# ErlerPhilipp/points2surf

Measured on NVIDIA H100. Metric: SDF queries/sec at grid_res=256, higher is better.
Workload: dtype f16 operands / f32 accumulate (wgmma); hi/lo split f16 (fp32-level) for FC tails and guard-band recompute

## Files before the change

### points2surf_b200/csrc/net_tc.cu

```cuda
#include "model.cuh"
#include "tc_ptx.cuh"

namespace p2s {

using namespace ptx;

namespace {

constexpr int kTile = 64;
constexpr int kWG = 2;
constexpr int kThreads = 128 * kWG;
template <bool PRECISE>
struct Cfg {
    static constexpr int kChunks = PRECISE ? 2 : 4;
    static constexpr int kSplit = 8 / kChunks;
    static constexpr uint32_t kChunkBytes = PRECISE ? 65536u : 32768u;
    static constexpr uint32_t kW3Bytes = kChunks * kChunkBytes;
    static constexpr uint32_t kMidScale = PRECISE ? 2u : 1u;
    static constexpr uint32_t kMidBytes = (8192u + 8192u + 16384u) * kMidScale;
    static constexpr uint32_t kPerqBytes = PRECISE ? 16384u : 8192u;
    static constexpr uint32_t kRedBytes = 4u * kChunks * 128u * 4u;
    static constexpr uint32_t kOffMid = kW3Bytes;
    static constexpr uint32_t kWgWq = kPerqBytes;
    static constexpr uint32_t kWgBytes = kWgWq + 192 * 4;
    static constexpr uint32_t kOffWg = kOffMid + kMidBytes;
    static constexpr uint32_t kOffBias = kOffWg + kWG * kWgBytes;
    static constexpr uint32_t kSlotBytes = PRECISE ? 0u : 8u * 128u * 16u;
    static constexpr uint32_t kOffSlot = kOffBias + 320 * 4;
    static constexpr uint32_t kOffXBar = kOffSlot + kWG * kSlotBytes;
    static constexpr uint32_t kSmemBytes = kOffXBar + (PRECISE ? 0u : kWG * 16u);
};
static_assert(Cfg<false>::kSmemBytes <= 232448 && Cfg<true>::kSmemBytes <= 232448, "shared memory budget");
static_assert(Cfg<false>::kRedBytes <= Cfg<false>::kPerqBytes && Cfg<true>::kRedBytes <= Cfg<true>::kPerqBytes, "reduction scratch");

struct Seg {
    const float* ptr;
    int n;
    int tiles;
    int center;
};

struct PassParams {
    Seg seg[2];
    const float* query;
    const float* R;
    int tiles_per_query;
    int B;
    const float* W0;
    const float* b0;
    int num_mid;
    int mid_N[3];
    const uint8_t* mid_img[3];
    const float* mid_bias[3];
    int perq_layer;
    const uint8_t* perq_img;
    const uint8_t* w3_img;
    float* out;
};

__device__ __forceinline__ uint32_t pack_relu(float a, float b) {
    uint32_t r;
    asm("cvt.rn.relu.satfinite.f16x2.f32 %0, %1, %2;" : "=r"(r) : "f"(b), "f"(a));
    return r;
}
__device__ __forceinline__ void pack_relu_split(float a, float b, uint32_t& hi, uint32_t& lo) {
    hi = pack_relu(a, b);
    const float2 hf = __half22float2(*reinterpret_cast<const __half2*>(&hi));
    lo = pack_half2(fmaxf(a, 0.f) - hf.x, fmaxf(b, 0.f) - hf.y);
}
template <bool PRECISE>
__device__ __forceinline__ void pack_act(float a, float b, uint32_t& hi, uint32_t& lo) {
    if (PRECISE) pack_relu_split(a, b, hi, lo);
    else hi = pack_relu(a, b);
}

template <bool PRECISE, int R>
__device__ __forceinline__ void mid_mma(float (&d)[R], const uint32_t (&a)[4], const uint32_t (&al)[4], uint64_t w, uint64_t w_lo, uint32_t acc) {
    if (R == 32) {
        auto& d32 = reinterpret_cast<float (&)[32]>(d);
        if (PRECISE) { wgmma_rs_n64(d32, al, w, acc); wgmma_rs_n64(d32, a, w_lo, 1); wgmma_rs_n64(d32, a, w, 1); }
        else wgmma_rs_n64(d32, a, w, acc);
    } else {
        auto& d64 = reinterpret_cast<float (&)[64]>(d);
        if (PRECISE) { wgmma_rs_n128(d64, al, w, acc); wgmma_rs_n128(d64, a, w_lo, 1); wgmma_rs_n128(d64, a, w, 1); }
        else wgmma_rs_n128(d64, a, w, acc);
    }
}

template <bool PRECISE, int R, int KL>
__device__ __forceinline__ void pack_acc(const float (&d)[R], const float* bias, int q4, uint32_t (&a)[R / 8][4], uint32_t (&al)[R / 8][KL]) {
#pragma unroll
    for (int j = 0; j < R / 4; ++j) {
        const float2 bb = *reinterpret_cast<const float2*>(bias + 8 * j + 2 * q4);
        pack_act<PRECISE>(d[4 * j] + bb.x, d[4 * j + 1] + bb.y, a[j >> 1][(j & 1) * 2], al[j >> 1][PRECISE ? (j & 1) * 2 : 0]);
        pack_act<PRECISE>(d[4 * j + 2] + bb.x, d[4 * j + 3] + bb.y, a[j >> 1][(j & 1) * 2 + 1], al[j >> 1][PRECISE ? (j & 1) * 2 + 1 : 0]);
    }
}

template <int S>
__device__ __forceinline__ void max_halve(float (&m)[32], int lane) {
    const bool up = (lane & S) != 0;
#pragma unroll
    for (int i = 0; i < S; ++i) {
        const float send = up ? m[i] : m[i + S], keep = up ? m[i + S] : m[i];
        m[i] = fmaxf(keep, __shfl_xor_sync(0xffffffffu, send, S));
    }
}

template <bool PRECISE>
__global__ void __launch_bounds__(kThreads, 1) pointnet_pass_kernel(const PassParams p) {
    using C = Cfg<PRECISE>;
    constexpr int kL = PRECISE ? 4 : 1;
    extern __shared__ __align__(1024) uint8_t smem[];
    float* s_bias = reinterpret_cast<float*>(smem + C::kOffBias);
    const int tid = threadIdx.x, wg = tid >> 7, t = tid & 127, lane = tid & 31, q4 = lane & 3;
    const int r0 = (t >> 5) * 16 + (lane >> 2);
    const int part = blockIdx.x % C::kSplit;
    const int stream = blockIdx.x / C::kSplit, nstreams = gridDim.x / C::kSplit;
    const int nq = (p.B > stream) ? (p.B - stream + nstreams - 1) / nstreams : 0;
    const int tpq = p.tiles_per_query;
    uint32_t mid_off[3] = {0, 0, 0};
    {
        uint32_t o = 0;
        for (int l = 0; l < (PRECISE ? p.num_mid : 3); ++l) {
            if (!PRECISE && l >= p.num_mid) break;
            mid_off[l] = o; o += (uint32_t)p.mid_N[l] * 128u * C::kMidScale;
        }
    }

    if (nq > 0) {
        const uint4* src = reinterpret_cast<const uint4*>(p.w3_img + (size_t)part * C::kW3Bytes);
        uint4* dst = reinterpret_cast<uint4*>(smem);
        for (uint32_t i = tid; i < C::kW3Bytes / 16; i += kThreads) dst[i] = src[i];
        for (int l = 0; l < (PRECISE ? p.num_mid : 3); ++l) {
            if (!PRECISE && l >= p.num_mid) break;
            if (l == p.perq_layer) continue;
            const uint4* s = reinterpret_cast<const uint4*>(p.mid_img[l]);
            uint4* d = reinterpret_cast<uint4*>(smem + C::kOffMid + mid_off[l]);
            for (uint32_t i = tid; i < (uint32_t)p.mid_N[l] * 8u * C::kMidScale; i += kThreads) d[i] = s[i];
        }
    }
    {
        int off = 0;
        for (int l = 0; l < p.num_mid; ++l) {
            for (int i = tid; i < p.mid_N[l]; i += kThreads) s_bias[off + i] = p.mid_bias[l][i];
            off += p.mid_N[l];
        }
        for (int i = tid; i < 64; i += kThreads) s_bias[256 + i] = p.b0[i];
    }
    uint64_t* xbar = reinterpret_cast<uint64_t*>(smem + C::kOffXBar);
    if (!PRECISE && tid == 0) {
        for (int w = 0; w < kWG; ++w) {
            mbar_init(xbar + 2 * w, 1);
            mbar_arrive_expect_tx(xbar + 2 * w, C::kSlotBytes);
            mbar_init(xbar + 2 * w + 1, 128);
        }
        fence_mbar_init();
    }
    fence_proxy_async_smem();
    __syncthreads();
    if (!PRECISE) cluster_sync();

    uint8_t* wsm = smem + C::kOffWg + wg * C::kWgBytes;
    uint8_t* perq = wsm;
    float* red = reinterpret_cast<float*>(perq);
    float* wq = reinterpret_cast<float*>(wsm + C::kWgWq);
    const float* s_b0 = s_bias + 256;
    const uint32_t bar_id = 1 + (uint32_t)wg;
    auto wg_sync = [&]() { asm volatile("bar.sync %0, 128;" ::"r"(bar_id) : "memory"); };
    const uint64_t dsc_w3 = make_smem_desc(smem_u32(smem), 128, 2048);
    uint64_t dsc_mid[3], dsc_mid_lo[3];
    for (int l = 0; l < 3; ++l) {
        const bool pq = l == p.perq_layer;
        dsc_mid[l] = make_smem_desc(pq ? smem_u32(perq) : smem_u32(smem + C::kOffMid) + mid_off[l], 128, 1024);
        dsc_mid_lo[l] = dsc_mid[l] + (uint64_t)((pq ? 8192u : (uint32_t)p.mid_N[l] * 128u) >> 4);
    }
    uint8_t* slot = smem + C::kOffSlot + wg * C::kSlotBytes;
    uint64_t* full = xbar + 2 * wg;
    uint64_t* empty = xbar + 2 * wg + 1;
    const uint32_t peer = (uint32_t)part ^ 1u;
    uint32_t nsend = 0, nrecv = 0;

    for (int qi = wg; qi < nq; qi += kWG) {
        const size_t q = (size_t)stream + (size_t)qi * nstreams;
        wg_sync();
        if (t < 64) {
            const float w0 = p.W0[t * 3 + 0], w1 = p.W0[t * 3 + 1], w2 = p.W0[t * 3 + 2];
            float r[9] = {1.f, 0.f, 0.f, 0.f, 1.f, 0.f, 0.f, 0.f, 1.f};
            if (p.R) {
#pragma unroll
                for (int i = 0; i < 9; ++i) r[i] = p.R[q * 9 + i];
            }
            wq[0 * 64 + t] = w0 * r[0] + w1 * r[3] + w2 * r[6];
            wq[1 * 64 + t] = w0 * r[1] + w1 * r[4] + w2 * r[7];
            wq[2 * 64 + t] = w0 * r[2] + w1 * r[5] + w2 * r[8];
        }
        if (p.perq_layer >= 0) {
            const uint4* s = reinterpret_cast<const uint4*>(p.perq_img + q * C::kPerqBytes);
            uint4* d = reinterpret_cast<uint4*>(perq);
            for (uint32_t i = t; i < C::kPerqBytes / 16; i += 128) d[i] = s[i];
            fence_proxy_async_smem();
        }
        wg_sync();
        float vmax[4 * C::kChunks];
#pragma unroll
        for (int i = 0; i < 4 * C::kChunks; ++i) vmax[i] = -INFINITY;
        const int own = PRECISE ? 0 : (part ^ wg ^ (qi >> 1)) & 1;
        for (int i = 0; i < tpq; ++i) {
            const int tq = PRECISE ? i : (i & ~1) + own;
            const bool mine = PRECISE || (!(i & 1) && tq < tpq);
            uint32_t a2[8][4], a2l[8][kL];
            if (mine) {
                const int sgi = tq < p.seg[0].tiles ? 0 : 1;
                const Seg& sg = p.seg[sgi];
                float cx = 0.f, cy = 0.f, cz = 0.f;
                if (sg.center) { cx = p.query[q * 3 + 0]; cy = p.query[q * 3 + 1]; cz = p.query[q * 3 + 2]; }
                float px[2], py[2], pz[2];
#pragma unroll
                for (int h = 0; h < 2; ++h) {
                    int local = (tq - (sgi ? p.seg[0].tiles : 0)) * kTile + r0 + 8 * h;
                    if (local >= sg.n) local = 0;
                    const float* src = sg.ptr + (q * sg.n + local) * 3;
                    px[h] = src[0] - cx; py[h] = src[1] - cy; pz[h] = src[2] - cz;
                }
                uint32_t a[4][4], al[4][kL];
#pragma unroll
                for (int kk = 0; kk < 4; ++kk) {
#pragma unroll
                    for (int hc = 0; hc < 2; ++hc) {
                        const int ch = kk * 16 + hc * 8 + 2 * q4;
                        const float2 wx = *reinterpret_cast<const float2*>(wq + 0 * 64 + ch);
                        const float2 wy = *reinterpret_cast<const float2*>(wq + 1 * 64 + ch);
                        const float2 wz = *reinterpret_cast<const float2*>(wq + 2 * 64 + ch);
                        const float2 bb = *reinterpret_cast<const float2*>(s_b0 + ch);
#pragma unroll
                        for (int h = 0; h < 2; ++h) {
                            const float v0 = fmaf(wx.x, px[h], fmaf(wy.x, py[h], fmaf(wz.x, pz[h], bb.x)));
                            const float v1 = fmaf(wx.y, px[h], fmaf(wy.y, py[h], fmaf(wz.y, pz[h], bb.y)));
                            pack_act<PRECISE>(v0, v1, a[kk][hc * 2 + h], al[kk][PRECISE ? hc * 2 + h : 0]);
                        }
                    }
                }
                const float* bl = s_bias;
#pragma unroll
                for (int l = 0; l < 2; ++l) {
                    if (l >= p.num_mid - 1) break;
                    float d[32];
#pragma unroll
                    for (int i = 0; i < 32; ++i) d[i] = 0.f;
                    wgmma_fence();
#pragma unroll
                    for (int ks = 0; ks < 4; ++ks)
                        mid_mma<PRECISE>(d, a[ks], reinterpret_cast<const uint32_t (&)[4]>(al[PRECISE ? ks : 0]), dsc_mid[l] + (uint64_t)(ks * 16), dsc_mid_lo[l] + (uint64_t)(ks * 16), ks > 0);
                    wgmma_commit();
                    wgmma_wait<0>();
                    fence_regs(d);
                    pack_acc<PRECISE>(d, bl, q4, a, al);
                    bl += 64;
                }
                {
                    const uint64_t w = p.num_mid == 3 ? dsc_mid[2] : dsc_mid[0], w_lo = p.num_mid == 3 ? dsc_mid_lo[2] : dsc_mid_lo[0];
                    float d[64];
#pragma unroll
                    for (int i = 0; i < 64; ++i) d[i] = 0.f;
                    wgmma_fence();
#pragma unroll
                    for (int ks = 0; ks < 4; ++ks)
                        mid_mma<PRECISE>(d, a[ks], reinterpret_cast<const uint32_t (&)[4]>(al[PRECISE ? ks : 0]), w + (uint64_t)(ks * 16), w_lo + (uint64_t)(ks * 16), ks > 0);
                    wgmma_commit();
                    wgmma_wait<0>();
                    fence_regs(d);
                    pack_acc<PRECISE>(d, bl, q4, a2, a2l);
                }
                if (!PRECISE) {
                    if (nsend > 0) mbar_wait_cluster_bounded(empty, (nsend - 1) & 1);
                    const uint32_t dst = mapa(smem_u32(slot), peer) + 16u * (uint32_t)t, bar = mapa(smem_u32(full), peer);
#pragma unroll
                    for (int k = 0; k < 8; ++k) st_async_v4(dst + 2048u * k, a2[k], bar);
                    ++nsend;
                }
            } else {
                mbar_wait_cluster_bounded(full, nrecv & 1);
#pragma unroll
                for (int k = 0; k < 8; ++k) {
                    const uint4 v = reinterpret_cast<const uint4*>(slot)[128 * k + t];
                    a2[k][0] = v.x; a2[k][1] = v.y; a2[k][2] = v.z; a2[k][3] = v.w;
                }
                mbar_arrive_cluster(mapa(smem_u32(empty), peer));
                if (t == 0) mbar_arrive_expect_tx(full, C::kSlotBytes);
                ++nrecv;
            }
#pragma unroll(PRECISE ? 1 : C::kChunks)
            for (int c = 0; c < C::kChunks; ++c) {
                float d[64];
#pragma unroll
                for (int i = 0; i < 64; ++i) d[i] = 0.f;
                const uint64_t w = dsc_w3 + (uint64_t)((uint32_t)c * (C::kChunkBytes >> 4));
                wgmma_fence();
#pragma unroll
                for (int ks = 0; ks < 8; ++ks) {
                    const uint64_t o = w + (uint64_t)(ks * 16);
                    if (PRECISE) {
                        wgmma_rs_n128(d, a2[ks], o + (uint64_t)(32768u >> 4), ks > 0);
                        wgmma_rs_n128(d, reinterpret_cast<const uint32_t (&)[4]>(a2l[PRECISE ? ks : 0]), o, 1);
                        wgmma_rs_n128(d, a2[ks], o, 1);
                    } else {
                        wgmma_rs_n128(d, a2[ks], o, ks > 0);
                    }
                }
                wgmma_commit();
                wgmma_wait<0>();
                fence_regs(d);
                float m[32];
#pragma unroll
                for (int j = 0; j < 16; ++j) {
                    m[2 * j] = fmaxf(d[4 * j], d[4 * j + 2]);
                    m[2 * j + 1] = fmaxf(d[4 * j + 1], d[4 * j + 3]);
                }
                max_halve<16>(m, lane);
                max_halve<8>(m, lane);
                max_halve<4>(m, lane);
                float v[4];
#pragma unroll
                for (int i = 0; i < 4; ++i) v[i] = fmaxf(vmax[i], m[i]);
#pragma unroll
                for (int i = 0; i < 4 * (C::kChunks - 1); ++i) vmax[i] = vmax[i + 4];
#pragma unroll
                for (int i = 0; i < 4; ++i) vmax[4 * (C::kChunks - 1) + i] = v[i];
            }
        }
        constexpr int kC = C::kChunks * 128;
        const int warp = t >> 5;
        wg_sync();
#pragma unroll
        for (int c = 0; c < C::kChunks; ++c)
#pragma unroll
            for (int h = 0; h < 2; ++h)
                *reinterpret_cast<float2*>(red + warp * kC + c * 128 + 16 * (lane >> 2) + 8 * h + 2 * q4) = make_float2(vmax[4 * c + 2 * h], vmax[4 * c + 2 * h + 1]);
        wg_sync();
        for (int i = t; i < kC / 4; i += 128) {
            const float4* r4 = reinterpret_cast<const float4*>(red);
            float4 v = r4[i];
#pragma unroll
            for (int w = 1; w < 4; ++w) {
                const float4 u = r4[w * (kC / 4) + i];
                v = make_float4(fmaxf(v.x, u.x), fmaxf(v.y, u.y), fmaxf(v.z, u.z), fmaxf(v.w, u.w));
            }
            *reinterpret_cast<float4*>(p.out + q * 1024 + (size_t)(part * kC + 4 * i)) = v;
        }
    }
    if (!PRECISE) cluster_sync();
}

__global__ void pack_kmajor_kernel(const float* __restrict__ W, int rows, int K, int row0, uint32_t sbo, uint8_t* __restrict__ img, int lo) {
    int e = blockIdx.x * blockDim.x + threadIdx.x;
    if (e >= rows * K) return;
    int r = e / K, k = e % K;
    uint32_t off = (uint32_t)(r >> 3) * sbo + (uint32_t)(k >> 3) * 128u + (uint32_t)(r & 7) * 16u + (uint32_t)(k & 7) * 2u;
    const float w = W[(size_t)(row0 + r) * K + k];
    const __half h = __float2half_rn(w);
    *reinterpret_cast<__half*>(img + off) = lo ? __float2half_rn(w - __half2float(h)) : h;
}

__global__ void pack_perq_kernel(const float* __restrict__ W, int64_t B, uint8_t* __restrict__ img) {
    int64_t e = (int64_t)blockIdx.x * blockDim.x + threadIdx.x;
    if (e >= B * 4096) return;
    int64_t b = e >> 12;
    int r = (int)((e >> 6) & 63), k = (int)(e & 63);
    uint32_t off = (uint32_t)(r >> 3) * 1024u + (uint32_t)(k >> 3) * 128u + (uint32_t)(r & 7) * 16u + (uint32_t)(k & 7) * 2u;
    *reinterpret_cast<__half*>(img + b * 8192 + off) = __float2half_rn(W[e]);
}

__global__ void __launch_bounds__(256) fold_w1_kernel(const float* __restrict__ W1, const float* __restrict__ T, int64_t B, uint8_t* __restrict__ img) {
    __shared__ float sW[64][65];
    __shared__ __align__(16) float sT[64][68];
    const int64_t b = blockIdx.x;
    const int tid = threadIdx.x;
    for (int e = tid; e < 4096; e += 256) {
        const int r = e >> 6, c = e & 63;
        sW[r][c] = W1[e];
        sT[r][c] = T[b * 4096 + e] + (r == c ? 1.0f : 0.0f);
    }
    __syncthreads();
    const int o = tid >> 2, i0 = (tid & 3) * 16;
    float acc[16];
#pragma unroll
    for (int i = 0; i < 16; ++i) acc[i] = 0.f;
    for (int j = 0; j < 64; ++j) {
        const float w = sW[o][j];
#pragma unroll
        for (int i4 = 0; i4 < 4; ++i4) {
            const float4 t4 = *reinterpret_cast<const float4*>(&sT[j][i0 + 4 * i4]);
            acc[4 * i4 + 0] = fmaf(w, t4.x, acc[4 * i4 + 0]);
            acc[4 * i4 + 1] = fmaf(w, t4.y, acc[4 * i4 + 1]);
            acc[4 * i4 + 2] = fmaf(w, t4.z, acc[4 * i4 + 2]);
            acc[4 * i4 + 3] = fmaf(w, t4.w, acc[4 * i4 + 3]);
        }
    }
    uint8_t* dst = img + b * 8192 + (uint32_t)(o >> 3) * 1024u + (uint32_t)(o & 7) * 16u;
#pragma unroll
    for (int h = 0; h < 2; ++h) {
        uint32_t v[4];
#pragma unroll
        for (int e = 0; e < 4; ++e) v[e] = pack_half2(acc[h * 8 + 2 * e], acc[h * 8 + 2 * e + 1]);
        *reinterpret_cast<uint4*>(dst + (uint32_t)(i0 / 8 + h) * 128u) = make_uint4(v[0], v[1], v[2], v[3]);
    }
}

__global__ void fold_fc3_kernel(const float* __restrict__ W1, const float* __restrict__ Wfc3, const float* __restrict__ bfc3,
                                float* __restrict__ G, float* __restrict__ g0) {
    const int oi = blockIdx.x;
    const int o = oi >> 6, i = oi & 63;
    const int k = threadIdx.x;
    float acc = 0.f;
    for (int j = 0; j < 64; ++j) acc = fmaf(W1[o * 64 + j], Wfc3[(size_t)(j * 64 + i) * 256 + k], acc);
    G[(size_t)oi * 256 + k] = acc;
    if (k == 0) {
        float b = W1[o * 64 + i];
        for (int j = 0; j < 64; ++j) b = fmaf(W1[o * 64 + j], bfc3[j * 64 + i], b);
        g0[oi] = b;
    }
}

__global__ void transpose64_kernel(const float* __restrict__ in, float* __restrict__ out, int64_t B) {
    int64_t e = (int64_t)blockIdx.x * blockDim.x + threadIdx.x;
    if (e >= B * 4096) return;
    int64_t b = e >> 12;
    int i = (int)((e >> 6) & 63), j = (int)(e & 63);
    out[e] = in[b * 4096 + j * 64 + i];
}

__global__ void guard_flag_kernel(const float* __restrict__ logits, int od, int64_t B, float band, int32_t* __restrict__ list, int* __restrict__ count, int64_t base, int64_t cap) {
    int64_t i = (int64_t)blockIdx.x * blockDim.x + threadIdx.x;
    if (i >= B) return;
// ... 18 lines not shown
    if (e >= (int64_t)n * row_floats) return;
    int i = (int)(e / row_floats), j = (int)(e % row_floats);
    dst[(int64_t)list[i] * row_floats + j] = src[e];
}

}

struct TcStack {
    uint8_t* w3_img = nullptr;
    uint8_t* mid_img[3] = {nullptr, nullptr, nullptr};
    uint8_t* w3_img_p = nullptr;
    uint8_t* mid_img_p[3] = {nullptr, nullptr, nullptr};
    const float* mid_bias[3] = {nullptr, nullptr, nullptr};
    int mid_N[3] = {0, 0, 0};
    int num_mid = 0;
    const float* W0 = nullptr;
    const float* b0 = nullptr;
    const float* b3 = nullptr;
};

struct TcFc {
    const Layer* L = nullptr;
    const uint8_t* img = nullptr;
};
struct TcStnFc { TcFc fc1, fc2, fc3; };

struct TcWeights {
    TcStack qstn;
    TcStack stn[2], fin[2];
    TcStnFc qstn_fc, stn_fc[2];
    TcFc head_fc1[2], head_fc2, head_fc3;
    const uint8_t* fold_img[2] = {nullptr, nullptr};
    const float* fold_bias[2] = {nullptr, nullptr};
    TcStack stn_enc, fin_enc;
    TcStnFc stn_fc_enc;
    TcFc head_fc1_enc;
    const uint8_t* fold_img_enc = nullptr;
    const float* fold_bias_enc = nullptr;
    bool fc_on_tc = true;
    std::vector<void*> allocs;
    int sm_count = 132;
    int pass_clusters = 66;
    bool prof_on = false;
    std::vector<std::pair<cudaEvent_t, cudaEvent_t>> prof_events;
    double prof_flops = 0.0;
    ~TcWeights() {
        for (void* a : allocs) cudaFree(a);
        for (auto& e : prof_events) { cudaEventDestroy(e.first); cudaEventDestroy(e.second); }
    }
};

namespace {

uint8_t* tc_alloc(TcWeights& t, size_t bytes) {
    void* p = nullptr;
    P2S_CUDA(cudaMalloc(&p, bytes));
    P2S_CUDA(cudaMemset(p, 0, bytes));
    t.allocs.push_back(p);
    return (uint8_t*)p;
}

uint8_t* pack_layer(TcWeights& t, const Layer& L, uint32_t sbo, bool split = false) {
    const size_t one = (size_t)L.cout * L.cin * 2;
    uint8_t* img = tc_alloc(t, one * (split ? 2 : 1));
    P2S_LAUNCH(pack_kmajor_kernel, (unsigned)cdiv((int64_t)L.cout * L.cin, 256), 256, 0, 0, L.W, L.cout, L.cin, 0, sbo, img, 0);
    if (split) P2S_LAUNCH(pack_kmajor_kernel, (unsigned)cdiv((int64_t)L.cout * L.cin, 256), 256, 0, 0, L.W, L.cout, L.cin, 0, sbo, img + one, 1);
    return img;
}

uint8_t* pack_w3(TcWeights& t, const Layer& L, bool split = false) {
    P2S_CHECK(L.cout == 1024 && L.cin == 128, "big layer must be 128 -> 1024");
    const size_t chunk = split ? 65536 : 32768;
    uint8_t* img = tc_alloc(t, 8 * chunk);
    for (int c = 0; c < 8; ++c) {
        P2S_LAUNCH(pack_kmajor_kernel, (unsigned)cdiv(128 * 128, 256), 256, 0, 0, L.W, 128, 128, c * 128, 2048u, img + (size_t)c * chunk, 0);
        if (split) P2S_LAUNCH(pack_kmajor_kernel, (unsigned)cdiv(128 * 128, 256), 256, 0, 0, L.W, 128, 128, c * 128, 2048u, img + (size_t)c * chunk + 32768, 1);
    }
    return img;
}

cudaLaunchConfig_t pass_cluster_config(int grid, cudaStream_t st, cudaLaunchAttribute (&attr)[1]) {
    cudaLaunchConfig_t cfg{};
    cfg.gridDim = dim3((unsigned)grid);
    cfg.blockDim = dim3(kThreads);
    cfg.dynamicSmemBytes = Cfg<false>::kSmemBytes;
    cfg.stream = st;
    attr[0].id = cudaLaunchAttributeClusterDimension;
    attr[0].val.clusterDim.x = 2;
    attr[0].val.clusterDim.y = 1;
    attr[0].val.clusterDim.z = 1;
    cfg.attrs = attr;
    cfg.numAttrs = 1;
    return cfg;
}

void launch_pass(Model& m, const TcStack& s, const Seg& s0, const Seg& s1, const float* query, const float* R,
                 int64_t B, int perq_layer, const uint8_t* perq_img, float* out, cudaStream_t st, bool precise) {
    PassParams p{};
    p.seg[0] = s0; p.seg[1] = s1;
    p.query = query; p.R = R;
    p.tiles_per_query = s0.tiles + s1.tiles;
    p.B = (int)B;
    p.W0 = s.W0; p.b0 = s.b0;
    p.num_mid = s.num_mid;
    for (int l = 0; l < 3; ++l) { p.mid_N[l] = s.mid_N[l]; p.mid_img[l] = precise ? s.mid_img_p[l] : s.mid_img[l]; p.mid_bias[l] = s.mid_bias[l]; }
    p.perq_layer = perq_layer;
    p.perq_img = perq_img;
    p.w3_img = precise ? s.w3_img_p : s.w3_img;
    p.out = out;
    for (int l = 0; l < s.num_mid; ++l)
        P2S_CHECK(s.mid_N[l] == (l == s.num_mid - 1 ? 128 : 64), "pass kernel: mid layers must be 64 -> 64 ... -> 128");
    TcWeights& t = *m.tc;
    const int split = precise ? Cfg<true>::kSplit : Cfg<false>::kSplit;
    int streams = precise ? t.sm_count / split : t.pass_clusters;
    if ((int64_t)streams > B) streams = (int)B;
    const int grid = streams * split;
    cudaEvent_t e0 = nullptr, e1 = nullptr;
    const bool prof = t.prof_on && !precise;
    if (prof) {
        P2S_CUDA(cudaEventCreate(&e0)); P2S_CUDA(cudaEventCreate(&e1));
        P2S_CUDA(cudaEventRecord(e0, st));
    }
    if (precise) P2S_LAUNCH(pointnet_pass_kernel<true>, grid, kThreads, Cfg<true>::kSmemBytes, st, p);
    else {
        cudaLaunchAttribute cluster[1];
        const cudaLaunchConfig_t cfg = pass_cluster_config(grid, st, cluster);
        P2S_CUDA(cudaLaunchKernelEx(&cfg, pointnet_pass_kernel<false>, p));
        g_launches.fetch_add(1, std::memory_order_relaxed);
    }
    if (prof) {
        P2S_CUDA(cudaEventRecord(e1, st));
        t.prof_events.emplace_back(e0, e1);
        double mac_pt = 3.0 * 64 + 128.0 * 1024;
        int prev = 64;
        for (int l = 0; l < s.num_mid; ++l) { mac_pt += (double)prev * s.mid_N[l]; prev = s.mid_N[l]; }
        t.prof_flops += 2.0 * mac_pt * (double)(s0.n + s1.n) * (double)B;
    }
}

Seg make_seg(const float* ptr, int n, int center) { return Seg{ptr, n, n > 0 ? (n + kTile - 1) / kTile : 0, center}; }

void run_fc(const TcFc& f, const float* in, int lda, float* out, int ldc, int64_t Bc, bool relu, bool on_tc, cudaStream_t st,
            const float* in_bias = nullptr, bool in_relu = false) {
    const Layer& L = *f.L;
    if (on_tc && f.img) launch_fc_tc(in, lda, f.img, L.b, out, ldc, Bc, L.cout, L.cin, relu, st, 0, in_bias, in_relu);
    else {
        P2S_CHECK(!in_bias, "input bias needs the tensor-core FC kernel");
        launch_gemm_nt(in, 0, lda, L.W, 0, L.b, out, 0, ldc, (int)Bc, L.cout, L.cin, 1, relu, st);
    }
}

void fc_tail(const Layer& b3src, const TcStnFc& s, bool on_tc, const float* gmax_raw, int64_t Bc, float* g, float* f1, float* f2, float* out, cudaStream_t st) {
    if (on_tc && s.fc1.img) run_fc(s.fc1, gmax_raw, 1024, f1, 512, Bc, true, true, st, b3src.b, true);
    else {
        P2S_CUDA(cudaMemcpyAsync(g, gmax_raw, (size_t)Bc * 1024 * 4, cudaMemcpyDeviceToDevice, st));
        launch_bias_act(g, b3src.b, Bc, 1024, true, st);
        run_fc(s.fc1, g, 1024, f1, 512, Bc, true, on_tc, st);
    }
    run_fc(s.fc2, f1, 512, f2, 256, Bc, true, on_tc, st);
    run_fc(s.fc3, f2, 256, out, s.fc3.L->cout, Bc, false, on_tc, st);
}

}

void tc_build(Model& m) {
    P2S_CHECK(m.cfg.net_size == 1024, "tensor-core path needs net_size 1024");
    TcWeights* t = new TcWeights();
    m.tc = t;
    cudaDeviceProp prop;
    P2S_CUDA(cudaGetDeviceProperties(&prop, m.device));
    t->sm_count = prop.multiProcessorCount;
    P2S_CUDA(cudaFuncSetAttribute(pointnet_pass_kernel<false>, cudaFuncAttributeMaxDynamicSharedMemorySize, (int)Cfg<false>::kSmemBytes));
    P2S_CUDA(cudaFuncSetAttribute(pointnet_pass_kernel<true>, cudaFuncAttributeMaxDynamicSharedMemorySize, (int)Cfg<true>::kSmemBytes));
    {
        cudaLaunchAttribute cluster[1];
        const cudaLaunchConfig_t cfg = pass_cluster_config(2 * (t->sm_count / 2), 0, cluster);
        int clusters = 0;
        P2S_CUDA(cudaOccupancyMaxActiveClusters(&clusters, pointnet_pass_kernel<false>, &cfg));
        P2S_CHECK(clusters > 0, "pass kernel: no cluster of two CTAs fits on the device");
        t->pass_clusters = std::min(clusters, t->sm_count / 2);
    }
    auto build_stn = [&](TcStack& s, const Stn& stn, const Layer* c0a, const Layer* c0b) {
        if (!c0a) {
            s.W0 = stn.c1.W; s.b0 = stn.c1.b;
            s.num_mid = 1;
            s.mid_img[0] = pack_layer(*t, stn.c2, 1024); s.mid_bias[0] = stn.c2.b; s.mid_N[0] = 128;
            s.mid_img_p[0] = pack_layer(*t, stn.c2, 1024, true);
        } else {
            s.W0 = c0a->W; s.b0 = c0a->b;
            s.num_mid = 3;
            s.mid_img[0] = pack_layer(*t, *c0b, 1024); s.mid_bias[0] = c0b->b; s.mid_N[0] = 64;
            s.mid_img[1] = pack_layer(*t, stn.c1, 1024); s.mid_bias[1] = stn.c1.b; s.mid_N[1] = 64;
            s.mid_img[2] = pack_layer(*t, stn.c2, 1024); s.mid_bias[2] = stn.c2.b; s.mid_N[2] = 128;
            s.mid_img_p[0] = pack_layer(*t, *c0b, 1024, true);
            s.mid_img_p[1] = pack_layer(*t, stn.c1, 1024, true);
            s.mid_img_p[2] = pack_layer(*t, stn.c2, 1024, true);
        }
        s.w3_img_p = pack_w3(*t, stn.c3, true);
        s.w3_img = pack_w3(*t, stn.c3);
        s.b3 = stn.c3.b;
    };
    auto build_fin = [&](TcStack& s, const Feat& f) {
        s.W0 = f.conv0a.W; s.b0 = f.conv0a.b;
        s.num_mid = 3;
        s.mid_img[0] = pack_layer(*t, f.conv0b, 1024); s.mid_bias[0] = f.conv0b.b; s.mid_N[0] = 64;
        s.mid_img[1] = nullptr; s.mid_bias[1] = f.conv1.b; s.mid_N[1] = 64;
// ... 255 lines not shown
```

Measured before the change: 431,100.

## Warp-specialize fast pass kernel into producer and two consumer warpgroups

```diff
diff --git a/points2surf_b200/csrc/net_tc.cu b/points2surf_b200/csrc/net_tc.cu
--- a/points2surf_b200/csrc/net_tc.cu
+++ b/points2surf_b200/csrc/net_tc.cu
@@ -8,10 +8,10 @@
 namespace {
 
 constexpr int kTile = 64;
-constexpr int kWG = 2;
-constexpr int kThreads = 128 * kWG;
 template <bool PRECISE>
 struct Cfg {
+    static constexpr int kWG = PRECISE ? 2 : 3;
+    static constexpr int kThreads = 128 * kWG;
     static constexpr int kChunks = PRECISE ? 2 : 4;
     static constexpr int kSplit = 8 / kChunks;
     static constexpr uint32_t kChunkBytes = PRECISE ? 65536u : 32768u;
@@ -19,19 +19,25 @@
     static constexpr uint32_t kMidScale = PRECISE ? 2u : 1u;
     static constexpr uint32_t kMidBytes = (8192u + 8192u + 16384u) * kMidScale;
     static constexpr uint32_t kPerqBytes = PRECISE ? 16384u : 8192u;
-    static constexpr uint32_t kRedBytes = 4u * kChunks * 128u * 4u;
+    static constexpr int kRedChunks = PRECISE ? kChunks : kChunks / 2;
+    static constexpr uint32_t kRedBytes = 4u * kRedChunks * 128u * 4u;
     static constexpr uint32_t kOffMid = kW3Bytes;
+    static constexpr int kQueryWG = PRECISE ? 2 : 1;
     static constexpr uint32_t kWgWq = kPerqBytes;
     static constexpr uint32_t kWgBytes = kWgWq + 192 * 4;
     static constexpr uint32_t kOffWg = kOffMid + kMidBytes;
-    static constexpr uint32_t kOffBias = kOffWg + kWG * kWgBytes;
+    static constexpr uint32_t kOffBias = kOffWg + kQueryWG * kWgBytes;
+    static constexpr uint32_t kOffRed = kOffBias + 320 * 4;
     static constexpr uint32_t kSlotBytes = PRECISE ? 0u : 8u * 128u * 16u;
-    static constexpr uint32_t kOffSlot = kOffBias + 320 * 4;
-    static constexpr uint32_t kOffXBar = kOffSlot + kWG * kSlotBytes;
-    static constexpr uint32_t kSmemBytes = kOffXBar + (PRECISE ? 0u : kWG * 16u);
+    static constexpr uint32_t kOffOwn = kOffRed + (PRECISE ? 0u : 2u * kRedBytes);
+    static constexpr uint32_t kOffPeer = kOffOwn + kSlotBytes;
+    static constexpr uint32_t kOffBar = kOffPeer + kSlotBytes;
+    static constexpr uint32_t kSmemBytes = kOffBar + (PRECISE ? 0u : 5u * 8u);
 };
 static_assert(Cfg<false>::kSmemBytes <= 232448 && Cfg<true>::kSmemBytes <= 232448, "shared memory budget");
-static_assert(Cfg<false>::kRedBytes <= Cfg<false>::kPerqBytes && Cfg<true>::kRedBytes <= Cfg<true>::kPerqBytes, "reduction scratch");
+static_assert(Cfg<true>::kRedBytes <= Cfg<true>::kPerqBytes, "reduction scratch");
+static_assert(Cfg<false>::kOffOwn % 16 == 0 && Cfg<false>::kOffBar % 8 == 0, "slot / mbarrier alignment");
+enum XBar { kOwnFull, kOwnEmpty, kPeerFull, kConsumed, kPeerEmpty };
 
 struct Seg {
     const float* ptr;
@@ -107,65 +113,212 @@
     }
 }
 
+template <bool PRECISE> constexpr int kLo = PRECISE ? 4 : 1;
+
 template <bool PRECISE>
-__global__ void __launch_bounds__(kThreads, 1) pointnet_pass_kernel(const PassParams p) {
+__device__ __forceinline__ void mid_offsets(const PassParams& p, uint32_t (&mid_off)[3]) {
+    uint32_t o = 0;
+    mid_off[0] = mid_off[1] = mid_off[2] = 0;
+    for (int l = 0; l < (PRECISE ? p.num_mid : 3); ++l) {
+        if (!PRECISE && l >= p.num_mid) break;
+        mid_off[l] = o; o += (uint32_t)p.mid_N[l] * 128u * Cfg<PRECISE>::kMidScale;
+    }
+}
+
+template <bool PRECISE>
+__device__ __forceinline__ void load_resident(const PassParams& p, uint8_t* smem, int part, bool any, const uint32_t (&mid_off)[3]) {
     using C = Cfg<PRECISE>;
-    constexpr int kL = PRECISE ? 4 : 1;
-    extern __shared__ __align__(1024) uint8_t smem[];
+    const int tid = threadIdx.x;
     float* s_bias = reinterpret_cast<float*>(smem + C::kOffBias);
-    const int tid = threadIdx.x, wg = tid >> 7, t = tid & 127, lane = tid & 31, q4 = lane & 3;
-    const int r0 = (t >> 5) * 16 + (lane >> 2);
-    const int part = blockIdx.x % C::kSplit;
-    const int stream = blockIdx.x / C::kSplit, nstreams = gridDim.x / C::kSplit;
-    const int nq = (p.B > stream) ? (p.B - stream + nstreams - 1) / nstreams : 0;
-    const int tpq = p.tiles_per_query;
-    uint32_t mid_off[3] = {0, 0, 0};
-    {
-        uint32_t o = 0;
-        for (int l = 0; l < (PRECISE ? p.num_mid : 3); ++l) {
-            if (!PRECISE && l >= p.num_mid) break;
-            mid_off[l] = o; o += (uint32_t)p.mid_N[l] * 128u * C::kMidScale;
-        }
-    }
-
-    if (nq > 0) {
+    if (any) {
         const uint4* src = reinterpret_cast<const uint4*>(p.w3_img + (size_t)part * C::kW3Bytes);
         uint4* dst = reinterpret_cast<uint4*>(smem);
-        for (uint32_t i = tid; i < C::kW3Bytes / 16; i += kThreads) dst[i] = src[i];
+        for (uint32_t i = tid; i < C::kW3Bytes / 16; i += C::kThreads) dst[i] = src[i];
         for (int l = 0; l < (PRECISE ? p.num_mid : 3); ++l) {
             if (!PRECISE && l >= p.num_mid) break;
             if (l == p.perq_layer) continue;
             const uint4* s = reinterpret_cast<const uint4*>(p.mid_img[l]);
             uint4* d = reinterpret_cast<uint4*>(smem + C::kOffMid + mid_off[l]);
-            for (uint32_t i = tid; i < (uint32_t)p.mid_N[l] * 8u * C::kMidScale; i += kThreads) d[i] = s[i];
-        }
-    }
-    {
-        int off = 0;
-        for (int l = 0; l < p.num_mid; ++l) {
-            for (int i = tid; i < p.mid_N[l]; i += kThreads) s_bias[off + i] = p.mid_bias[l][i];
-            off += p.mid_N[l];
-        }
-        for (int i = tid; i < 64; i += kThreads) s_bias[256 + i] = p.b0[i];
-    }
-    uint64_t* xbar = reinterpret_cast<uint64_t*>(smem + C::kOffXBar);
-    if (!PRECISE && tid == 0) {
-        for (int w = 0; w < kWG; ++w) {
-            mbar_init(xbar + 2 * w, 1);
-            mbar_arrive_expect_tx(xbar + 2 * w, C::kSlotBytes);
-            mbar_init(xbar + 2 * w + 1, 128);
-        }
-        fence_mbar_init();
-    }
+            for (uint32_t i = tid; i < (uint32_t)p.mid_N[l] * 8u * C::kMidScale; i += C::kThreads) d[i] = s[i];
+        }
+    }
+    int off = 0;
+    for (int l = 0; l < p.num_mid; ++l) {
+        for (int i = tid; i < p.mid_N[l]; i += C::kThreads) s_bias[off + i] = p.mid_bias[l][i];
+        off += p.mid_N[l];
+    }
+    for (int i = tid; i < 64; i += C::kThreads) s_bias[256 + i] = p.b0[i];
+}
+
+template <bool PRECISE>
+__device__ __forceinline__ void query_setup(const PassParams& p, size_t q, int t, float* wq, uint8_t* perq) {
+    if (t < 64) {
+        const float w0 = p.W0[t * 3 + 0], w1 = p.W0[t * 3 + 1], w2 = p.W0[t * 3 + 2];
+        float r[9] = {1.f, 0.f, 0.f, 0.f, 1.f, 0.f, 0.f, 0.f, 1.f};
+        if (p.R) {
+#pragma unroll
+            for (int i = 0; i < 9; ++i) r[i] = p.R[q * 9 + i];
+        }
+        wq[0 * 64 + t] = w0 * r[0] + w1 * r[3] + w2 * r[6];
+        wq[1 * 64 + t] = w0 * r[1] + w1 * r[4] + w2 * r[7];
+        wq[2 * 64 + t] = w0 * r[2] + w1 * r[5] + w2 * r[8];
+    }
+    if (p.perq_layer >= 0) {
+        const uint4* s = reinterpret_cast<const uint4*>(p.perq_img + q * Cfg<PRECISE>::kPerqBytes);
+        uint4* d = reinterpret_cast<uint4*>(perq);
+        for (uint32_t i = t; i < Cfg<PRECISE>::kPerqBytes / 16; i += 128) d[i] = s[i];
+        fence_proxy_async_smem();
+    }
+}
+
+__device__ __forceinline__ void load_points(const PassParams& p, size_t q, int tq, int r0, float (&pt)[6]) {
+    const int sgi = tq < p.seg[0].tiles ? 0 : 1;
+    const Seg& sg = p.seg[sgi];
+    float cx = 0.f, cy = 0.f, cz = 0.f;
+    if (sg.center) { cx = p.query[q * 3 + 0]; cy = p.query[q * 3 + 1]; cz = p.query[q * 3 + 2]; }
+#pragma unroll
+    for (int h = 0; h < 2; ++h) {
+        int local = (tq - (sgi ? p.seg[0].tiles : 0)) * kTile + r0 + 8 * h;
+        if (local >= sg.n) local = 0;
+        const float* src = sg.ptr + (q * sg.n + local) * 3;
+        pt[h] = src[0] - cx; pt[2 + h] = src[1] - cy; pt[4 + h] = src[2] - cz;
+    }
+}
+
+template <bool PRECISE>
+__device__ __forceinline__ void tile_layers(const PassParams& p, const float (&pt)[6], const float* wq, const float* s_bias, int q4,
+                                            const uint64_t (&dsc_mid)[3], const uint64_t (&dsc_mid_lo)[3],
+                                            uint32_t (&a2)[8][4], uint32_t (&a2l)[8][kLo<PRECISE>]) {
+    const float* s_b0 = s_bias + 256;
+    uint32_t a[4][4], al[4][kLo<PRECISE>];
+#pragma unroll
+    for (int kk = 0; kk < 4; ++kk) {
+#pragma unroll
+        for (int hc = 0; hc < 2; ++hc) {
+            const int ch = kk * 16 + hc * 8 + 2 * q4;
+            const float2 wx = *reinterpret_cast<const float2*>(wq + 0 * 64 + ch);
+            const float2 wy = *reinterpret_cast<const float2*>(wq + 1 * 64 + ch);
+            const float2 wz = *reinterpret_cast<const float2*>(wq + 2 * 64 + ch);
+            const float2 bb = *reinterpret_cast<const float2*>(s_b0 + ch);
+#pragma unroll
+            for (int h = 0; h < 2; ++h) {
+                const float v0 = fmaf(wx.x, pt[h], fmaf(wy.x, pt[2 + h], fmaf(wz.x, pt[4 + h], bb.x)));
+                const float v1 = fmaf(wx.y, pt[h], fmaf(wy.y, pt[2 + h], fmaf(wz.y, pt[4 + h], bb.y)));
+                pack_act<PRECISE>(v0, v1, a[kk][hc * 2 + h], al[kk][PRECISE ? hc * 2 + h : 0]);
+            }
+        }
+    }
+    const float* bl = s_bias;
+#pragma unroll
+    for (int l = 0; l < 2; ++l) {
+        if (l >= p.num_mid - 1) break;
+        float d[32];
+#pragma unroll
+        for (int i = 0; i < 32; ++i) d[i] = 0.f;
+        wgmma_fence();
+#pragma unroll
+        for (int ks = 0; ks < 4; ++ks)
+            mid_mma<PRECISE>(d, a[ks], reinterpret_cast<const uint32_t (&)[4]>(al[PRECISE ? ks : 0]), dsc_mid[l] + (uint64_t)(ks * 16), dsc_mid_lo[l] + (uint64_t)(ks * 16), ks > 0);
+        wgmma_commit();
+        wgmma_wait<0>();
+        fence_regs(d);
+        pack_acc<PRECISE>(d, bl, q4, a, al);
+        bl += 64;
+    }
+    const uint64_t w = p.num_mid == 3 ? dsc_mid[2] : dsc_mid[0], w_lo = p.num_mid == 3 ? dsc_mid_lo[2] : dsc_mid_lo[0];
+    float d[64];
+#pragma unroll
+    for (int i = 0; i < 64; ++i) d[i] = 0.f;
+    wgmma_fence();
+#pragma unroll
+    for (int ks = 0; ks < 4; ++ks)
+        mid_mma<PRECISE>(d, a[ks], reinterpret_cast<const uint32_t (&)[4]>(al[PRECISE ? ks : 0]), w + (uint64_t)(ks * 16), w_lo + (uint64_t)(ks * 16), ks > 0);
+    wgmma_commit();
+    wgmma_wait<0>();
+    fence_regs(d);
+    pack_acc<PRECISE>(d, bl, q4, a2, a2l);
+}
+
+template <bool PRECISE, typename WaitTurn, typename PassTurn>
+__device__ __forceinline__ void chunk_max(const uint32_t (&a2)[8][4], const uint32_t (&a2l)[8][kLo<PRECISE>], uint64_t w, int lane, float (&vm)[4],
+                                          WaitTurn wait_turn, PassTurn pass_turn) {
+    float d[64];
+#pragma unroll
+    for (int i = 0; i < 64; ++i) d[i] = 0.f;
+    wait_turn();
+    wgmma_fence();
+#pragma unroll
+    for (int ks = 0; ks < 8; ++ks) {
+        const uint64_t o = w + (uint64_t)(ks * 16);
+        if (PRECISE) {
+            wgmma_rs_n128(d, a2[ks], o + (uint64_t)(32768u >> 4), ks > 0);
+            wgmma_rs_n128(d, reinterpret_cast<const uint32_t (&)[4]>(a2l[PRECISE ? ks : 0]), o, 1);
+            wgmma_rs_n128(d, a2[ks], o, 1);
+        } else {
+            wgmma_rs_n128(d, a2[ks], o, ks > 0);
+        }
+    }
+    wgmma_commit();
+    pass_turn();
+    wgmma_wait<0>();
+    fence_regs(d);
+    float m[32];
+#pragma unroll
+    for (int j = 0; j < 16; ++j) {
+        m[2 * j] = fmaxf(d[4 * j], d[4 * j + 2]);
+        m[2 * j + 1] = fmaxf(d[4 * j + 1], d[4 * j + 3]);
+    }
+    max_halve<16>(m, lane);
+    max_halve<8>(m, lane);
+    max_halve<4>(m, lane);
+#pragma unroll
+    for (int i = 0; i < 4; ++i) vm[i] = fmaxf(vm[i], m[i]);
+}
+
+template <int kCh, typename Sync>
+__device__ __forceinline__ void store_max(const float (&vmax)[4 * kCh], float* red, int t, Sync sync, float* out) {
+    constexpr int kC = kCh * 128;
+    const int warp = t >> 5, lane = t & 31, q4 = lane & 3;
+    sync();
+#pragma unroll
+    for (int c = 0; c < kCh; ++c)
+#pragma unroll
+        for (int h = 0; h < 2; ++h)
+            *reinterpret_cast<float2*>(red + warp * kC + c * 128 + 16 * (lane >> 2) + 8 * h + 2 * q4) = make_float2(vmax[4 * c + 2 * h], vmax[4 * c + 2 * h + 1]);
+    sync();
+    for (int i = t; i < kC / 4; i += 128) {
+        const float4* r4 = reinterpret_cast<const float4*>(red);
+        float4 v = r4[i];
+#pragma unroll
+        for (int w = 1; w < 4; ++w) {
+            const float4 u = r4[w * (kC / 4) + i];
+            v = make_float4(fmaxf(v.x, u.x), fmaxf(v.y, u.y), fmaxf(v.z, u.z), fmaxf(v.w, u.w));
+        }
+        *reinterpret_cast<float4*>(out + 4 * i) = v;
+    }
+}
+
+__device__ __forceinline__ void pass_precise(const PassParams& p) {
+    using C = Cfg<true>;
+    constexpr int kL = kLo<true>;
+    extern __shared__ __align__(1024) uint8_t smem[];
+    const float* s_bias = reinterpret_cast<const float*>(smem + C::kOffBias);
+    const int tid = threadIdx.x, wg = tid >> 7, t = tid & 127, lane = tid & 31, q4 = lane & 3;
+    const int part = blockIdx.x % C::kSplit;
+    const int stream = blockIdx.x / C::kSplit, nstreams = gridDim.x / C::kSplit;
+    const int nq = (p.B > stream) ? (p.B - stream + nstreams - 1) / nstreams : 0;
+    const int tpq = p.tiles_per_query;
+    const int r0 = (t >> 5) * 16 + (lane >> 2);
+    uint32_t mid_off[3];
+    mid_offsets<true>(p, mid_off);
+    load_resident<true>(p, smem, part, nq > 0, mid_off);
     fence_proxy_async_smem();
     __syncthreads();
-    if (!PRECISE) cluster_sync();
 
     uint8_t* wsm = smem + C::kOffWg + wg * C::kWgBytes;
     uint8_t* perq = wsm;
     float* red = reinterpret_cast<float*>(perq);
     float* wq = reinterpret_cast<float*>(wsm + C::kWgWq);
-    const float* s_b0 = s_bias + 256;
     const uint32_t bar_id = 1 + (uint32_t)wg;
     auto wg_sync = [&]() { asm volatile("bar.sync %0, 128;" ::"r"(bar_id) : "memory"); };
     const uint64_t dsc_w3 = make_smem_desc(smem_u32(smem), 128, 2048);
@@ -175,181 +328,184 @@
         dsc_mid[l] = make_smem_desc(pq ? smem_u32(perq) : smem_u32(smem + C::kOffMid) + mid_off[l], 128, 1024);
         dsc_mid_lo[l] = dsc_mid[l] + (uint64_t)((pq ? 8192u : (uint32_t)p.mid_N[l] * 128u) >> 4);
     }
-    uint8_t* slot = smem + C::kOffSlot + wg * C::kSlotBytes;
-    uint64_t* full = xbar + 2 * wg;
-    uint64_t* empty = xbar + 2 * wg + 1;
-    const uint32_t peer = (uint32_t)part ^ 1u;
-    uint32_t nsend = 0, nrecv = 0;
-
-    for (int qi = wg; qi < nq; qi += kWG) {
+
+    for (int qi = wg; qi < nq; qi += C::kWG) {
         const size_t q = (size_t)stream + (size_t)qi * nstreams;
         wg_sync();
-        if (t < 64) {
-            const float w0 = p.W0[t * 3 + 0], w1 = p.W0[t * 3 + 1], w2 = p.W0[t * 3 + 2];
-            float r[9] = {1.f, 0.f, 0.f, 0.f, 1.f, 0.f, 0.f, 0.f, 1.f};
-            if (p.R) {
-#pragma unroll
-                for (int i = 0; i < 9; ++i) r[i] = p.R[q * 9 + i];
-            }
-            wq[0 * 64 + t] = w0 * r[0] + w1 * r[3] + w2 * r[6];
-            wq[1 * 64 + t] = w0 * r[1] + w1 * r[4] + w2 * r[7];
-            wq[2 * 64 + t] = w0 * r[2] + w1 * r[5] + w2 * r[8];
-        }
-        if (p.perq_layer >= 0) {
-            const uint4* s = reinterpret_cast<const uint4*>(p.perq_img + q * C::kPerqBytes);
-            uint4* d = reinterpret_cast<uint4*>(perq);
-            for (uint32_t i = t; i < C::kPerqBytes / 16; i += 128) d[i] = s[i];
-            fence_proxy_async_smem();
-        }
+        query_setup<true>(p, q, t, wq, perq);
         wg_sync();
         float vmax[4 * C::kChunks];
 #pragma unroll
         for (int i = 0; i < 4 * C::kChunks; ++i) vmax[i] = -INFINITY;
-        const int own = PRECISE ? 0 : (part ^ wg ^ (qi >> 1)) & 1;
-        for (int i = 0; i < tpq; ++i) {
-            const int tq = PRECISE ? i : (i & ~1) + own;
-            const bool mine = PRECISE || (!(i & 1) && tq < tpq);
+        for (int tq = 0; tq < tpq; ++tq) {
+            float pt[6];
+            load_points(p, q, tq, r0, pt);
             uint32_t a2[8][4], a2l[8][kL];
-            if (mine) {
-                const int sgi = tq < p.seg[0].tiles ? 0 : 1;
-                const Seg& sg = p.seg[sgi];
-                float cx = 0.f, cy = 0.f, cz = 0.f;
-                if (sg.center) { cx = p.query[q * 3 + 0]; cy = p.query[q * 3 + 1]; cz = p.query[q * 3 + 2]; }
-                float px[2], py[2], pz[2];
-#pragma unroll
-                for (int h = 0; h < 2; ++h) {
-                    int local = (tq - (sgi ? p.seg[0].tiles : 0)) * kTile + r0 + 8 * h;
-                    if (local >= sg.n) local = 0;
-                    const float* src = sg.ptr + (q * sg.n + local) * 3;
-                    px[h] = src[0] - cx; py[h] = src[1] - cy; pz[h] = src[2] - cz;
-                }
-                uint32_t a[4][4], al[4][kL];
-#pragma unroll
-                for (int kk = 0; kk < 4; ++kk) {
-#pragma unroll
-                    for (int hc = 0; hc < 2; ++hc) {
-                        const int ch = kk * 16 + hc * 8 + 2 * q4;
-                        const float2 wx = *reinterpret_cast<const float2*>(wq + 0 * 64 + ch);
-                        const float2 wy = *reinterpret_cast<const float2*>(wq + 1 * 64 + ch);
-                        const float2 wz = *reinterpret_cast<const float2*>(wq + 2 * 64 + ch);
-                        const float2 bb = *reinterpret_cast<const float2*>(s_b0 + ch);
-#pragma unroll
-                        for (int h = 0; h < 2; ++h) {
-                            const float v0 = fmaf(wx.x, px[h], fmaf(wy.x, py[h], fmaf(wz.x, pz[h], bb.x)));
-                            const float v1 = fmaf(wx.y, px[h], fmaf(wy.y, py[h], fmaf(wz.y, pz[h], bb.y)));
-                            pack_act<PRECISE>(v0, v1, a[kk][hc * 2 + h], al[kk][PRECISE ? hc * 2 + h : 0]);
-                        }
-                    }
-                }
-                const float* bl = s_bias;
-#pragma unroll
-                for (int l = 0; l < 2; ++l) {
-                    if (l >= p.num_mid - 1) break;
-                    float d[32];
-#pragma unroll
-                    for (int i = 0; i < 32; ++i) d[i] = 0.f;
-                    wgmma_fence();
-#pragma unroll
-                    for (int ks = 0; ks < 4; ++ks)
-                        mid_mma<PRECISE>(d, a[ks], reinterpret_cast<const uint32_t (&)[4]>(al[PRECISE ? ks : 0]), dsc_mid[l] + (uint64_t)(ks * 16), dsc_mid_lo[l] + (uint64_t)(ks * 16), ks > 0);
-                    wgmma_commit();
-                    wgmma_wait<0>();
-                    fence_regs(d);
-                    pack_acc<PRECISE>(d, bl, q4, a, al);
-                    bl += 64;
-                }
-                {
-                    const uint64_t w = p.num_mid == 3 ? dsc_mid[2] : dsc_mid[0], w_lo = p.num_mid == 3 ? dsc_mid_lo[2] : dsc_mid_lo[0];
-                    float d[64];
-#pragma unroll
-                    for (int i = 0; i < 64; ++i) d[i] = 0.f;
-                    wgmma_fence();
-#pragma unroll
-                    for (int ks = 0; ks < 4; ++ks)
-                        mid_mma<PRECISE>(d, a[ks], reinterpret_cast<const uint32_t (&)[4]>(al[PRECISE ? ks : 0]), w + (uint64_t)(ks * 16), w_lo + (uint64_t)(ks * 16), ks > 0);
-                    wgmma_commit();
-                    wgmma_wait<0>();
-                    fence_regs(d);
-                    pack_acc<PRECISE>(d, bl, q4, a2, a2l);
-                }
-                if (!PRECISE) {
-                    if (nsend > 0) mbar_wait_cluster_bounded(empty, (nsend - 1) & 1);
-                    const uint32_t dst = mapa(smem_u32(slot), peer) + 16u * (uint32_t)t, bar = mapa(smem_u32(full), peer);
-#pragma unroll
-                    for (int k = 0; k < 8; ++k) st_async_v4(dst + 2048u * k, a2[k], bar);
-                    ++nsend;
-                }
-            } else {
-                mbar_wait_cluster_bounded(full, nrecv & 1);
-#pragma unroll
-                for (int k = 0; k < 8; ++k) {
-                    const uint4 v = reinterpret_cast<const uint4*>(slot)[128 * k + t];
-                    a2[k][0] = v.x; a2[k][1] = v.y; a2[k][2] = v.z; a2[k][3] = v.w;
-                }
-                mbar_arrive_cluster(mapa(smem_u32(empty), peer));
-                if (t == 0) mbar_arrive_expect_tx(full, C::kSlotBytes);
-                ++nrecv;
-            }
-#pragma unroll(PRECISE ? 1 : C::kChunks)
+            tile_layers<true>(p, pt, wq, s_bias, q4, dsc_mid, dsc_mid_lo, a2, a2l);
+#pragma unroll 1
             for (int c = 0; c < C::kChunks; ++c) {
-                float d[64];
-#pragma unroll
-                for (int i = 0; i < 64; ++i) d[i] = 0.f;
-                const uint64_t w = dsc_w3 + (uint64_t)((uint32_t)c * (C::kChunkBytes >> 4));
-                wgmma_fence();
-#pragma unroll
-                for (int ks = 0; ks < 8; ++ks) {
-                    const uint64_t o = w + (uint64_t)(ks * 16);
-                    if (PRECISE) {
-                        wgmma_rs_n128(d, a2[ks], o + (uint64_t)(32768u >> 4), ks > 0);
-                        wgmma_rs_n128(d, reinterpret_cast<const uint32_t (&)[4]>(a2l[PRECISE ? ks : 0]), o, 1);
-                        wgmma_rs_n128(d, a2[ks], o, 1);
-                    } else {
-                        wgmma_rs_n128(d, a2[ks], o, ks > 0);
-                    }
-                }
-                wgmma_commit();
-                wgmma_wait<0>();
-                fence_regs(d);
-                float m[32];
-#pragma unroll
-                for (int j = 0; j < 16; ++j) {
-                    m[2 * j] = fmaxf(d[4 * j], d[4 * j + 2]);
-                    m[2 * j + 1] = fmaxf(d[4 * j + 1], d[4 * j + 3]);
-                }
-                max_halve<16>(m, lane);
-                max_halve<8>(m, lane);
-                max_halve<4>(m, lane);
-                float v[4];
-#pragma unroll
-                for (int i = 0; i < 4; ++i) v[i] = fmaxf(vmax[i], m[i]);
+                float v[4] = {vmax[0], vmax[1], vmax[2], vmax[3]};
+                chunk_max<true>(a2, a2l, dsc_w3 + (uint64_t)((uint32_t)c * (C::kChunkBytes >> 4)), lane, v, [] {}, [] {});
 #pragma unroll
                 for (int i = 0; i < 4 * (C::kChunks - 1); ++i) vmax[i] = vmax[i + 4];
 #pragma unroll
                 for (int i = 0; i < 4; ++i) vmax[4 * (C::kChunks - 1) + i] = v[i];
             }
         }
-        constexpr int kC = C::kChunks * 128;
-        const int warp = t >> 5;
-        wg_sync();
-#pragma unroll
-        for (int c = 0; c < C::kChunks; ++c)
-#pragma unroll
-            for (int h = 0; h < 2; ++h)
-                *reinterpret_cast<float2*>(red + warp * kC + c * 128 + 16 * (lane >> 2) + 8 * h + 2 * q4) = make_float2(vmax[4 * c + 2 * h], vmax[4 * c + 2 * h + 1]);
-        wg_sync();
-        for (int i = t; i < kC / 4; i += 128) {
-            const float4* r4 = reinterpret_cast<const float4*>(red);
-            float4 v = r4[i];
-#pragma unroll
-            for (int w = 1; w < 4; ++w) {
-                const float4 u = r4[w * (kC / 4) + i];
-                v = make_float4(fmaxf(v.x, u.x), fmaxf(v.y, u.y), fmaxf(v.z, u.z), fmaxf(v.w, u.w));
+        store_max<C::kChunks>(vmax, red, t, wg_sync, p.out + q * 1024 + (size_t)part * (C::kChunks * 128));
+    }
+}
+
+__device__ __forceinline__ void pass_pair(const PassParams& p) {
+    using C = Cfg<false>;
+    extern __shared__ __align__(1024) uint8_t smem[];
+    const float* s_bias = reinterpret_cast<const float*>(smem + C::kOffBias);
+    const int tid = threadIdx.x, wg = tid >> 7, t = tid & 127, lane = tid & 31, q4 = lane & 3;
+    const int part = blockIdx.x % C::kSplit;
+    const int stream = blockIdx.x / C::kSplit, nstreams = gridDim.x / C::kSplit;
+    const int nq = (p.B > stream) ? (p.B - stream + nstreams - 1) / nstreams : 0;
+    const int tpq = p.tiles_per_query;
+    const uint32_t peer = (uint32_t)part ^ 1u;
+    uint32_t mid_off[3];
+    mid_offsets<false>(p, mid_off);
+    load_resident<false>(p, smem, part, nq > 0, mid_off);
+    uint64_t* xbar = reinterpret_cast<uint64_t*>(smem + C::kOffBar);
+    if (tid == 0) {
+        mbar_init(xbar + kOwnFull, 128);
+        mbar_init(xbar + kOwnEmpty, 256);
+        mbar_init(xbar + kPeerFull, 1);
+        mbar_arrive_expect_tx(xbar + kPeerFull, C::kSlotBytes);
+        mbar_init(xbar + kConsumed, 256);
+        mbar_init(xbar + kPeerEmpty, 1);
+        fence_mbar_init();
+    }
+    fence_proxy_async_smem();
+    __syncthreads();
+    cluster_sync();
+    uint8_t* own_slot = smem + C::kOffOwn;
+    uint8_t* peer_slot = smem + C::kOffPeer;
+
+    if (wg == 0) {
+        uint8_t* perq = smem + C::kOffWg;
+        float* wq = reinterpret_cast<float*>(smem + C::kOffWg + C::kWgWq);
+        auto wg_sync = [&]() { asm volatile("bar.sync 1, 128;" ::: "memory"); };
+        const int r0 = (t >> 5) * 16 + (lane >> 2);
+        uint64_t dsc_mid[3], dsc_mid_lo[3];
+        for (int l = 0; l < 3; ++l) {
+            dsc_mid[l] = make_smem_desc(l == p.perq_layer ? smem_u32(perq) : smem_u32(smem + C::kOffMid) + mid_off[l], 128, 1024);
+            dsc_mid_lo[l] = dsc_mid[l];
+        }
+        const uint32_t dst = mapa(smem_u32(peer_slot), peer) + 16u * (uint32_t)t, bar_full = mapa(smem_u32(xbar + kPeerFull), peer);
+        const uint32_t bar_empty = mapa(smem_u32(xbar + kPeerEmpty), peer);
+        int qi = 0, i = 0, nskip = 0;
+        auto seek = [&]() {
+            while (qi < nq) {
+                const int tq = (i & ~1) + ((part ^ qi) & 1);
+                if (!(i & 1) && tq < tpq) break;
+                ++nskip;
+                if (++i == tpq) { i = 0; ++qi; }
             }
-            *reinterpret_cast<float4*>(p.out + q * 1024 + (size_t)(part * kC + 4 * i)) = v;
-        }
-    }
-    if (!PRECISE) cluster_sync();
+        };
+        seek();
+        float pt[6];
+        if (qi < nq) load_points(p, (size_t)stream + (size_t)qi * nstreams, (i & ~1) + ((part ^ qi) & 1), r0, pt);
+        int setup_qi = -1;
+        uint32_t nsend = 0, nrel = 0;
+        while (qi < nq) {
+            const int cqi = qi;
+            const int release = nskip;
+            const float cur[6] = {pt[0], pt[1], pt[2], pt[3], pt[4], pt[5]};
+            nskip = 0;
+            if (++i == tpq) { i = 0; ++qi; }
+            seek();
+            if (cqi != setup_qi) {
+                wg_sync();
+                query_setup<false>(p, (size_t)stream + (size_t)cqi * nstreams, t, wq, perq);
+                wg_sync();
+                setup_qi = cqi;
+            }
+            if (qi < nq) load_points(p, (size_t)stream + (size_t)qi * nstreams, (i & ~1) + ((part ^ qi) & 1), r0, pt);
+            uint32_t a2[8][4], a2l[8][1];
+            tile_layers<false>(p, cur, wq, s_bias, q4, dsc_mid, dsc_mid_lo, a2, a2l);
+            if (nsend > 0) mbar_wait_bounded(xbar + kOwnEmpty, (nsend - 1) & 1);
+#pragma unroll
+            for (int k = 0; k < 8; ++k) reinterpret_cast<uint4*>(own_slot)[128 * k + t] = make_uint4(a2[k][0], a2[k][1], a2[k][2], a2[k][3]);
+            mbar_arrive(xbar + kOwnFull);
+            if (t == 0) {
+                for (int r = 0; r < release; ++r, ++nrel) {
+                    mbar_wait_bounded(xbar + kConsumed, nrel & 1);
+                    mbar_arrive_expect_tx(xbar + kPeerFull, C::kSlotBytes);
+                    mbar_arrive_cluster(bar_empty);
+                }
+            }
+            if (nsend > 0) mbar_wait_cluster_bounded(xbar + kPeerEmpty, (nsend - 1) & 1);
+#pragma unroll
+            for (int k = 0; k < 8; ++k) st_async_v4(dst + 2048u * k, a2[k], bar_full);
+            ++nsend;
+        }
+        if (t == 0) {
+            for (int r = 0; r < nskip; ++r, ++nrel) {
+                mbar_wait_bounded(xbar + kConsumed, nrel & 1);
+                mbar_arrive_expect_tx(xbar + kPeerFull, C::kSlotBytes);
+                mbar_arrive_cluster(bar_empty);
+            }
+        }
+    } else {
+        const int cw = wg - 1;
+        float* red = reinterpret_cast<float*>(smem + C::kOffRed + (uint32_t)cw * C::kRedBytes);
+        const uint32_t bar_id = 2 + (uint32_t)cw;
+        auto wg_sync = [&]() { asm volatile("bar.sync %0, 128;" ::"r"(bar_id) : "memory"); };
+        const uint64_t dsc_w3 = make_smem_desc(smem_u32(smem), 128, 2048) + (uint64_t)((uint32_t)(2 * cw) * (C::kChunkBytes >> 4));
+        const uint32_t turn_mine = 4 + (uint32_t)cw, turn_other = 5 - (uint32_t)cw;
+        auto wait_turn = [&]() { asm volatile("bar.sync %0, 256;" ::"r"(turn_mine) : "memory"); };
+        auto pass_turn = [&]() { asm volatile("bar.arrive %0, 256;" ::"r"(turn_other) : "memory"); };
+        if (cw == 1) pass_turn();
+        uint32_t nown = 0, nrecv = 0;
+        for (int qi = 0; qi < nq; ++qi) {
+            const size_t q = (size_t)stream + (size_t)qi * nstreams;
+            const int own = (part ^ qi) & 1;
+            float vmax[8];
+#pragma unroll
+            for (int j = 0; j < 8; ++j) vmax[j] = -INFINITY;
+            for (int i = 0; i < tpq; ++i) {
+                const int tq = (i & ~1) + own;
+                const bool mine = !(i & 1) && tq < tpq;
+                uint32_t a2[8][4], a2l[8][1];
+                if (mine) {
+                    mbar_wait_bounded(xbar + kOwnFull, nown & 1);
+#pragma unroll
+                    for (int k = 0; k < 8; ++k) {
+                        const uint4 v = reinterpret_cast<const uint4*>(own_slot)[128 * k + t];
+                        a2[k][0] = v.x; a2[k][1] = v.y; a2[k][2] = v.z; a2[k][3] = v.w;
+                    }
+                    mbar_arrive(xbar + kOwnEmpty);
+                    ++nown;
+                } else {
+                    mbar_wait_cluster_bounded(xbar + kPeerFull, nrecv & 1);
+#pragma unroll
+                    for (int k = 0; k < 8; ++k) {
+                        const uint4 v = reinterpret_cast<const uint4*>(peer_slot)[128 * k + t];
+                        a2[k][0] = v.x; a2[k][1] = v.y; a2[k][2] = v.z; a2[k][3] = v.w;
+                    }
+                    mbar_arrive(xbar + kConsumed);
+                    ++nrecv;
+                }
+#pragma unroll
+                for (int c = 0; c < 2; ++c)
+                    chunk_max<false>(a2, a2l, dsc_w3 + (uint64_t)((uint32_t)c * (C::kChunkBytes >> 4)), lane,
+                                     reinterpret_cast<float (&)[4]>(vmax[4 * c]), wait_turn, pass_turn);
+            }
+            store_max<2>(vmax, red, t, wg_sync, p.out + q * 1024 + (size_t)(part * 512 + cw * 256));
+        }
+        if (cw == 0) wait_turn();
+    }
+    cluster_sync();
+}
+
+template <bool PRECISE>
+__global__ void __launch_bounds__(Cfg<PRECISE>::kThreads, 1) pointnet_pass_kernel(const PassParams p) {
+    if constexpr (PRECISE) pass_precise(p);
+    else pass_pair(p);
 }
 
 __global__ void pack_kmajor_kernel(const float* __restrict__ W, int rows, int K, int row0, uint32_t sbo, uint8_t* __restrict__ img, int lo) {
@@ -534,7 +690,7 @@
 cudaLaunchConfig_t pass_cluster_config(int grid, cudaStream_t st, cudaLaunchAttribute (&attr)[1]) {
     cudaLaunchConfig_t cfg{};
     cfg.gridDim = dim3((unsigned)grid);
-    cfg.blockDim = dim3(kThreads);
+    cfg.blockDim = dim3(Cfg<false>::kThreads);
     cfg.dynamicSmemBytes = Cfg<false>::kSmemBytes;
     cfg.stream = st;
     attr[0].id = cudaLaunchAttributeClusterDimension;
@@ -573,7 +729,7 @@
         P2S_CUDA(cudaEventCreate(&e0)); P2S_CUDA(cudaEventCreate(&e1));
         P2S_CUDA(cudaEventRecord(e0, st));
     }
-    if (precise) P2S_LAUNCH(pointnet_pass_kernel<true>, grid, kThreads, Cfg<true>::kSmemBytes, st, p);
+    if (precise) P2S_LAUNCH(pointnet_pass_kernel<true>, grid, Cfg<true>::kThreads, Cfg<true>::kSmemBytes, st, p);
     else {
         cudaLaunchAttribute cluster[1];
         const cudaLaunchConfig_t cfg = pass_cluster_config(grid, st, cluster);
```

New measurement: 440,500 (median of 6 runs). +2.2%, better.
